# phylo42/IPK

Measured on AMD Instinct MI355X. Metric: scored phylo-k-mers/sec, higher is better.
Workload: dtype f32

## Files before the change

ipk_amd/csrc/dcla_device.hpp:

```cpp
#pragma once
#include <hip/hip_runtime.h>
#include <stdint.h>

namespace ipkgpu {

constexpr __host__ __device__ uint32_t ipow(uint32_t b, int e) { return e <= 0 ? 1u : b * ipow(b, e - 1); }
constexpr __host__ __device__ uint64_t ipow64(uint64_t b, int e) { return e <= 0 ? 1ull : b * ipow64(b, e - 1); }
constexpr __host__ __device__ uint32_t umin_c(uint32_t a, uint32_t b) { return a < b ? a : b; }
constexpr __host__ __device__ uint32_t umax_c(uint32_t a, uint32_t b) { return a > b ? a : b; }

constexpr uint32_t LIST_OVERFLOW = 0xFFFFFFFFu;

__host__ __device__ __forceinline__ uint32_t enc_score_bits(uint32_t u)
{
    return (u & 0x80000000u) ? ~u : (u | 0x80000000u);
}
__host__ __device__ __forceinline__ uint32_t dec_score_bits(uint32_t e)
{
    return (e & 0x80000000u) ? (e & 0x7fffffffu) : ~e;
}

__device__ __forceinline__ uint32_t lane_id() { return threadIdx.x & 63u; }
__device__ __forceinline__ uint64_t ballot64(bool p) { return __builtin_amdgcn_ballot_w64(p); }
__device__ __forceinline__ uint32_t to_sgpr(uint32_t x)
{
    uint32_t r;
    asm volatile("s_nop 0\n\tv_readfirstlane_b32 %0, %1" : "=s"(r) : "v"(x));
    return r;
}

typedef uint32_t u32x2_t __attribute__((ext_vector_type(2)));

#ifdef IPK_EXEC_ASSERT
__device__ unsigned int g_exec_violations;
#define IPK_ASSERT_FULL_EXEC() do { if (__builtin_amdgcn_ballot_w64(true) != ~0ull) atomicAdd(&g_exec_violations, 1u); } while (0)
#else
#define IPK_ASSERT_FULL_EXEC() ((void)0)
#endif

template <int IMM = 0>
__device__ __forceinline__ void store8_lanes(const void* uniform_base, uint32_t byte_off, uint32_t x, uint32_t y, uint64_t mask)
{
    u32x2_t data; data.x = x; data.y = y;
    IPK_ASSERT_FULL_EXEC();
    asm volatile("s_mov_b64 exec, %3\n\tglobal_store_dwordx2 %0, %1, %2 offset:%4\n\ts_mov_b64 exec, -1"
                 : : "v"(byte_off), "v"(data), "s"(uniform_base), "s"(mask), "n"(IMM) : "memory");
}
template <int IMM = 0>
__device__ __forceinline__ void store4_lanes(const void* uniform_base, uint32_t byte_off, uint32_t x, uint64_t mask)
{
    IPK_ASSERT_FULL_EXEC();
    asm volatile("s_mov_b64 exec, %3\n\tglobal_store_dword %0, %1, %2 offset:%4\n\ts_mov_b64 exec, -1"
                 : : "v"(byte_off), "v"(x), "s"(uniform_base), "s"(mask), "n"(IMM) : "memory");
}

__device__ __forceinline__ uint32_t mbcnt(uint64_t mask)
{
    return __builtin_amdgcn_mbcnt_hi((uint32_t)(mask >> 32), __builtin_amdgcn_mbcnt_lo((uint32_t)mask, 0u));
}
__device__ __forceinline__ void wave_lds_sync()
{
    __builtin_amdgcn_fence(__ATOMIC_RELEASE, "wavefront");
    __builtin_amdgcn_wave_barrier();
    __builtin_amdgcn_fence(__ATOMIC_ACQUIRE, "wavefront");
}

struct WinCtx {
    const float* cols;
    const float* best;
    uint32_t w;
    uint32_t lead_c = 0;
};

template <int SIGMA, int J, int H>
struct Direct {
    static __device__ __forceinline__ bool eval(const WinCtx& c, float eps, uint32_t cand, float& score)
    {
        if constexpr (H == 1) {
            score = c.cols[(c.w + J) * SIGMA + cand];
            return score > eps;
        } else {
            constexpr int HL = H / 2, HR = H - HL;
            const float eps_l = eps - (c.best[c.w + J + H] - c.best[c.w + J + HL]);
            const float eps_r = eps - (c.best[c.w + J + HL] - c.best[c.w + J]);
            constexpr uint32_t PR = ipow(SIGMA, HR);
            const uint32_t cl = cand / PR, cr = cand - cl * PR;
            float sl, sr;
            const bool okl = Direct<SIGMA, J, HL>::eval(c, eps_l, cl, sl);
            const bool okr = Direct<SIGMA, J + HL, HR>::eval(c, eps_r, cr, sr);
            score = sl + sr;
            return okl & okr & (score > eps);
        }
    }
};

template <int SIGMA, int H, int CAP>
struct Geo {
    static constexpr uint64_t FULL = ipow64(SIGMA, H);
    static constexpr uint32_t CAPH = (uint32_t)(FULL < (uint64_t)CAP ? FULL : (uint64_t)CAP);
    static constexpr bool DIRECT = FULL <= 64;
    static constexpr int HL = H / 2, HR = H - H / 2;
    static constexpr uint32_t scratch()
    {
        if constexpr (DIRECT) return 0;
        else {
            using GL = Geo<SIGMA, HL, CAP>;
            using GR = Geo<SIGMA, HR, CAP>;
            return umax_c(GL::CAPH + GL::scratch(), GL::CAPH + GR::CAPH + GR::scratch());
        }
    }
    static constexpr uint32_t SCRATCH = scratch();
};

template <int SIGMA, int K, int CAP>
constexpr uint32_t wave_scratch_entries() { return Geo<SIGMA, K, CAP>::SCRATCH; }

__device__ __forceinline__ void divmod_u(uint32_t idx, uint32_t d, float rcp_d, uint32_t& q, uint32_t& r)
{
    q = (uint32_t)(((float)idx + 0.5f) * rcp_d);
    int32_t rem = (int32_t)idx - (int32_t)(q * d);
    if (rem < 0) { q -= 1; rem += (int32_t)d; }
    else if (rem >= (int32_t)d) { q += 1; rem -= (int32_t)d; }
    r = (uint32_t)rem;
}

template <class F>
__device__ __forceinline__ void for_each_pair(const uint2* L, uint32_t nL, const uint2* R, uint32_t nR, F&& f)
{
    const uint32_t lane = lane_id();
// ... 111 lines not shown
```

ipk_amd/csrc/ipkgpu.hip:

```cpp
#include <cstring>
#include <hip/hip_runtime.h>
#include <rocprim/rocprim.hpp>

#include <algorithm>
#include <cmath>
#include <cstdarg>
#include <cstdio>
#include <cstring>
#include <new>
#include <string>
#include <type_traits>
#include <unordered_map>
#include <memory>
#include <vector>

#include "../../include/ipkgpu.h"
#include "dcla_device.hpp"
#include "kernels_score.hpp"
#include "kernels_quad.hpp"
#include "kernels_compact.hpp"
#include "kernels_keymajor.hpp"
#include "kernels_reduce_pipe.hpp"
#include "kernels_filter.hpp"
#include "kernels_dbfile.hpp"
// ... 1910 lines not shown
        HIP_TRY(ctx, ctx_alloc(ctx, (void**)&e->d_entries, 8));
        if (positions) {
            Geometry geo;
            RC_TRY(fill_geometry(ctx, sigma, k, 0, geo));
            if (lead != 0 || geo.xp_nb == 0)
                return fail(ctx, IPKGPU_ERR_INVALID, "no positioned database for sigma=%u k=%u: the call takes the exact partition, which needs more than 64 keys "
                                                     "and no key-range pass", sigma, k);
            HIP_TRY(ctx, ctx_alloc(ctx, (void**)&e->d_positions, 4));
        }
        HIP_TRY(ctx, hipMemsetAsync(e->d_counts, 0, (size_t)n_owners * e->slots * 4, ctx->stream));
        HIP_TRY(ctx, hipStreamSynchronize(ctx->stream));
        eg.r = nullptr;
        *out = e;
        return IPKGPU_OK;
    }
    Plan pl;
    RC_TRY(make_plan(ctx, logp_dev, n_mats, sites, sigma, mat_group, k, log_eps, pl, lead, lead_c, false, positions));
    HIP_TRY(ctx, hipSetDevice(ctx->device));
    if (positions) {
        std::vector<uint32_t> rank(n_mats), seen(pl.n_groups, 0);
        for (uint32_t i = 0; i < n_mats; ++i) rank[i] = seen[pl.slot_of[i]]++;
        const uint32_t most = *std::max_element(seen.begin(), seen.end());
        if ((uint64_t)most * pl.nwin >= 0xFFFFFFFFull) return fail(ctx, IPKGPU_ERR_INVALID, "too many windows per group for the position code (%u matrices x %u windows)", most, pl.nwin);
        RC_TRY(ensure(ctx, ctx->mrank, (size_t)n_mats * 4));
        HIP_TRY(ctx, hipMemcpy(ctx->mrank.p, rank.data(), (size_t)n_mats * 4, hipMemcpyHostToDevice));
        pl.mat_rank = ctx->mrank.as<uint32_t>();
    }
    const uint64_t T = pl.table_size;
    const uint32_t P = n_owners;
    const uint64_t slots = (T + P - 1) / P;
    const uint32_t n_groups = pl.n_groups;

    ipkgpu_parts* parts = new (std::nothrow) ipkgpu_parts();
    if (!parts) return fail(ctx, IPKGPU_ERR_NOMEM, "out of host memory");
    parts->ctx = ctx; parts->n_owners = P; parts->slots = slots;
    parts->lead = lead; parts->key_base = key_base; parts->sigma = sigma; parts->k = k;
    parts->owner_off.assign((size_t)P + 1, 0);
    struct Guard { ipkgpu_parts* r; ~Guard() { if (r) ipkgpu_parts_free(r); } } guard{parts};

    RC_TRY(ensure(ctx, ctx->branch, (size_t)n_groups * 4));
    ctx->h_branch = pl.group_ids;
    HIP_TRY(ctx, hipMemcpyAsync(ctx->branch.p, ctx->h_branch.data(), (size_t)n_groups * 4, hipMemcpyHostToDevice, ctx->stream));

    ctx->acc_main_ms = ctx->acc_reduce_ms = ctx->acc_count_ms = ctx->acc_write_ms = ctx->acc_km_ms = 0;
    Stopwatch sw(ctx->stream, &ctx->events);
    const int t_begin = sw.mark();
    RC_TRY(run_prefix(ctx, pl, logp_dev));
    const int t_pre = sw.mark();
    std::vector<std::pair<int, int>> ev_score, ev_compact, ev_km;
    std::pair<int, int> ev_keys{-1, -1};

    struct Batch { uint32_t* counts = nullptr; uint2* entries = nullptr; uint2* pentries = nullptr; std::vector<uint64_t> owner_off; };
    std::vector<Batch> batches;
    auto free_batches = [&]() { for (auto& b : batches) { ctx_release(ctx, b.counts); ctx_release(ctx, b.entries); ctx_release(ctx, b.pentries); } batches.clear(); };
    struct BGuard { decltype(free_batches)& f; ~BGuard() { f(); } } bguard{free_batches};

    const uint64_t n_slots_all = (uint64_t)P * slots;
    uint32_t gpb_now = (uint32_t)pl.gpb, gb = 0;
    for (uint32_t g0 = 0; g0 < n_groups; g0 += gb) {
        gb = std::min<uint32_t>(gpb_now, n_groups - g0);
        const int s0 = sw.mark();
        const int rcb = score_batch(ctx, pl, logp_dev, g0, gb, &parts->emitted, true);
        if (rcb == IPKGPU_RETRY_SMALLER) { gpb_now = std::max<uint32_t>(1, gb / 2); gb = 0; continue; }
        if (rcb) return rcb;
        const int s1 = sw.mark();
        ev_score.push_back({s0, s1});
        parts->score_launches += 1;

        batches.emplace_back();
        Batch& b = batches.back();
        HIP_TRY(ctx, ctx_alloc(ctx, (void**)&b.counts, n_slots_all * 4));
        HIP_TRY(ctx, hipMemsetAsync(b.counts, 0, n_slots_all * 4, ctx->stream));
        const uint32_t kmc_pass = (uint32_t)std::min<int64_t>(256, std::max<int64_t>(4, ctx->opt_kmc_pass > 0 ? ctx->opt_kmc_pass : IPK_KMC_PASS));
        const bool fast_c = ctx->table_compressed && 64ull * (ctx->mask_words / 2) * 8 < (1ull << 32);
        uint32_t* qpack = nullptr;
        if (fast_c) {
            RC_TRY(ensure(ctx, ctx->qpack, n_slots_all * 4));
            if (gb <= kmc_pass) qpack = ctx->qpack.as<uint32_t>();
        }
        if (ctx->mask_valid && (T + 31) / 32 >= (uint64_t)ctx->num_cu * 1024)
            hipLaunchKernelGGL(km_count_mask_kernel, dim3((uint32_t)(((T + 31) / 32 + 255) / 256)), dim3(256), 0, ctx->stream,
                               ctx->mask.as<uint32_t>(), ctx->mask_words, T, gb, P, slots, b.counts, qpack);
        else if (ctx->mask_valid)
            hipLaunchKernelGGL(km_count_mask_key_kernel, dim3((uint32_t)((T + 255) / 256)), dim3(256), 0, ctx->stream,
                               ctx->mask.as<uint32_t>(), ctx->mask_words, T, gb, P, slots, b.counts, qpack);
        else
            hipLaunchKernelGGL(km_count_kernel, dim3((uint32_t)((T + 255) / 256)), dim3(256), 0, ctx->stream,
                               ctx->table.as<uint32_t>(), T, gb, P, slots, b.counts);
        HIP_TRY(ctx, hipGetLastError());
        RC_TRY(ensure(ctx, ctx->offsets, (n_slots_all + 1) * 8));
        RC_TRY(scan_u32(ctx, b.counts, n_slots_all, ctx->offsets.as<uint64_t>()));
        RC_TRY(ensure(ctx, ctx->goff, ((size_t)P + 1) * 8));
        hipLaunchKernelGGL(gather_offsets_kernel, dim3((P + 1 + 255) / 256), dim3(256), 0, ctx->stream,
                           ctx->offsets.as<uint64_t>(), (uint32_t)slots, P + 1, ctx->goff.as<uint64_t>());
        HIP_TRY(ctx, hipGetLastError());
        b.owner_off.resize((size_t)P + 1);
        const bool rb_ok = P <= RB_OWNERS_MAX;
        uint64_t* h_off = rb_ok ? reinterpret_cast<uint64_t*>(ctx->h_rb) + RB_OWNER_OFF : b.owner_off.data();
        HIP_TRY(ctx, hipMemcpyAsync(h_off, ctx->goff.p, ((size_t)P + 1) * 8, hipMemcpyDeviceToHost, ctx->stream));

        const bool pre_keys = P == 1 && g0 == 0 && gb == n_groups && rb_ok && !(ctx->opt_flags & 64) &&
                              (slots <= (1ull << 24) || ctx->last_entries * 8 >= slots * 12 * 4);
        uint32_t* k_keys = nullptr; uint64_t* k_off = nullptr;
        struct KGuard { ipkgpu_ctx* c; uint32_t*& a; uint64_t*& b; ~KGuard() { ctx_release(c, a); ctx_release(c, b); } } kguard{ctx, k_keys, k_off};
        int kt0 = -1, kt1 = -1;
        if (pre_keys) {
            kt0 = sw.mark();
            RC_TRY(ensure(ctx, ctx->tmp_b, (slots + 1) * 8));
            RC_TRY(scan_nonzero_u32(ctx, b.counts, slots, ctx->tmp_b.as<uint64_t>()));
            HIP_TRY(ctx, hipMemcpyAsync(h_off + P + 1, ctx->tmp_b.as<uint64_t>() + slots, 8, hipMemcpyDeviceToHost, ctx->stream));
            HIP_TRY(ctx, ctx_alloc(ctx, (void**)&k_keys, slots * 4));
            HIP_TRY(ctx, ctx_alloc(ctx, (void**)&k_off, (slots + 1) * 8));
            const uint32_t nbk = (uint32_t)((slots + 1 + 255) / 256);
            if (sigma == 4)
                hipLaunchKernelGGL(merge_write_keys_kernel<4>, dim3(nbk), dim3(256), 0, ctx->stream, b.counts, ctx->tmp_b.as<uint64_t>(),
                                   ctx->offsets.as<uint64_t>(), slots, (uint32_t)key_base, 1u, (int)k, k_keys, k_off);
            else
                hipLaunchKernelGGL(merge_write_keys_kernel<20>, dim3(nbk), dim3(256), 0, ctx->stream, b.counts, ctx->tmp_b.as<uint64_t>(),
                                   ctx->offsets.as<uint64_t>(), slots, 0u, 1u, (int)k, k_keys, k_off);
            HIP_TRY(ctx, hipGetLastError());
            kt1 = sw.mark();
        }

        uint2* w_dst = nullptr; bool w_posv = false;
        auto comp_table_w = [&]() { CompTable c = comp_table(ctx); if (w_posv) c.vaddr = ctx->pvaddr.as<uint64_t>(); return c; };
        auto launch_writer = [&](uint64_t cap_e) -> int {
            uint2* const dst_entries = w_dst ? w_dst : b.entries;
            if (ctx->table_compressed) {
                uint64_t per_xcd = (((T + 63) / 64) + 7) / 8;
                const uint32_t rows_now = qpack ? gb : std::min<uint32_t>(gb, kmc_pass);
                const bool runs = !(ctx->opt_flags & 4096) && IPK_KMC_RUNS_DEFAULT && (rows_now <= 128 || (ctx->opt_flags & 8192));
                if (runs && (qpack || fast_c)) per_xcd = (kmc_runs(T, ctx->comp_tbl) + 7) / 8;
                if (qpack && runs)
                    KM_LAUNCH(km_write_c_run_kernel, KMC_CAP, comp_table_w(), T, gb, ctx->branch.as<uint32_t>() + g0, P, slots, b.counts,
                              qpack, ctx->offsets.as<uint64_t>(), dst_entries, cap_e);
                else if (qpack)
                    KM_LAUNCH(km_write_c_kernel, KMC_CAP, comp_table_w(), T, gb, ctx->branch.as<uint32_t>() + g0, P, slots, b.counts,
                              qpack, ctx->offsets.as<uint64_t>(), dst_entries, cap_e);
                else if (fast_c) {
                    RC_TRY(ensure(ctx, ctx->pcounts, n_slots_all * 4));
                    for (uint32_t p0 = 0; p0 < gb; p0 += kmc_pass) {
                        const uint32_t pg = std::min<uint32_t>(kmc_pass, gb - p0);
                        const uint32_t* pmask = ctx->mask.as<uint32_t>() + (size_t)p0 * ctx->mask_words;
                        if ((T + 31) / 32 >= (uint64_t)ctx->num_cu * 1024)
                            hipLaunchKernelGGL(km_count_mask_kernel, dim3((uint32_t)(((T + 31) / 32 + 255) / 256)), dim3(256), 0, ctx->stream,
                                               pmask, ctx->mask_words, T, pg, P, slots, ctx->pcounts.as<uint32_t>(), ctx->qpack.as<uint32_t>());
                        else
                            hipLaunchKernelGGL(km_count_mask_key_kernel, dim3((uint32_t)((T + 255) / 256)), dim3(256), 0, ctx->stream,
                                               pmask, ctx->mask_words, T, pg, P, slots, ctx->pcounts.as<uint32_t>(), ctx->qpack.as<uint32_t>());
                        HIP_TRY(ctx, hipGetLastError());
                        CompTable ctp = comp_table_w();
                        ctp.mask = pmask;
                        ctp.vaddr += (size_t)p0 * (ctx->mask_words / 2);
                        ctp.rank += (size_t)p0 * (ctx->mask_words / 2);
                        if (runs)
                            KM_LAUNCH(km_write_c_run_kernel, KMC_CAP, ctp, T, pg, ctx->branch.as<uint32_t>() + g0 + p0, P, slots, ctx->pcounts.as<uint32_t>(),
                                      ctx->qpack.as<uint32_t>(), ctx->offsets.as<uint64_t>(), dst_entries, cap_e);
                        else
                            KM_LAUNCH(km_write_c_kernel, KMC_CAP, ctp, T, pg, ctx->branch.as<uint32_t>() + g0 + p0, P, slots, ctx->pcounts.as<uint32_t>(),
                                      ctx->qpack.as<uint32_t>(), ctx->offsets.as<uint64_t>(), dst_entries, cap_e);
                        HIP_TRY(ctx, hipGetLastError());
                    }
                } else if (positions)
                    return fail(ctx, IPKGPU_ERR_INVALID, "a positioned database of this many key slots per group would take the generic key-major writer, which carries no positions");
                else
                    hipLaunchKernelGGL(km_write_c_generic_kernel, dim3((uint32_t)((((T + 63) / 64 + 7) / 8) * 8)), dim3(256), 0, ctx->stream,
                                       comp_table(ctx), T, gb, ctx->branch.as<uint32_t>() + g0, P, slots,
                                       ctx->offsets.as<uint64_t>(), b.entries, cap_e);
            } else if ((ctx->opt_flags & 512) || (gb < 96 && !(ctx->opt_flags & 1024)))
                hipLaunchKernelGGL(km_write_kernel, dim3((uint32_t)((T + 63) / 64)), dim3(256), 0, ctx->stream,
                                   ctx->table.as<uint32_t>(), T, gb, ctx->branch.as<uint32_t>() + g0, P, slots,
                                   ctx->offsets.as<uint64_t>(), b.entries, cap_e);
            else
                hipLaunchKernelGGL(km_write_lines_kernel, dim3((uint32_t)((T + 63) / 64)), dim3(256), 0, ctx->stream,
                                   ctx->table.as<uint32_t>(), T, gb, ctx->branch.as<uint32_t>() + g0, P, slots,
                                   ctx->offsets.as<uint64_t>(), b.entries, cap_e);
            HIP_TRY(ctx, hipGetLastError());
            return IPKGPU_OK;
        };
        uint64_t cap_e = 0;
        const bool spec_e = rb_ok && ctx->last_gb > 0 && ctx->last_entries > 0 && !(ctx->opt_flags & 64) && !positions;
        int km0 = -1, km1 = -1;
        if (spec_e) {
            const uint64_t est = (uint64_t)((unsigned __int128)ctx->last_entries * gb / ctx->last_gb);
            size_t got = 0;
            if (ctx_alloc_atleast(ctx, (void**)&b.entries, est * 8, (est + est / 20 + 4096) * 8, &got) == hipSuccess) cap_e = got / 8;
            else { (void)hipGetLastError(); b.entries = nullptr; }
        }
        if (cap_e) { km0 = sw.mark(); RC_TRY(launch_writer(cap_e)); km1 = sw.mark(); }
        HIP_TRY(ctx, hipStreamSynchronize(ctx->stream));
        const int rcf = ctx->pend.active ? score_batch_finish(ctx, pl, g0, gb, &parts->emitted) : IPKGPU_OK;
        if (rcf == IPKGPU_RETRY_SMALLER || rcf == IPKGPU_RETRY_AGAIN) {
            ctx_release(ctx, b.counts); ctx_release(ctx, b.entries);
            batches.pop_back();
            ev_score.pop_back(); parts->score_launches -= 1;
            if (rcf == IPKGPU_RETRY_SMALLER) gpb_now = std::max<uint32_t>(1, gb / 2);
            gb = 0;
            continue;
        }
        if (rcf) return rcf;
        if (rb_ok) memcpy(b.owner_off.data(), h_off, ((size_t)P + 1) * 8);
        if (b.owner_off[P] > cap_e || cap_e == 0) {
            ctx_release(ctx, b.entries); b.entries = nullptr;
            HIP_TRY(ctx, ctx_alloc(ctx, (void**)&b.entries, std::max<uint64_t>(b.owner_off[P], 1) * 8));
            const uint64_t n_e = std::max<uint64_t>(b.owner_off[P], 1);
            km0 = sw.mark();
            if (positions) {
                if (!ctx->table_compressed) return fail(ctx, IPKGPU_ERR_INVALID, "internal: a positioned call ended in dense tables");
                const size_t cur_bytes = (n_slots_all + 1) * 8;
                RC_TRY(ensure(ctx, ctx->cursnap, cur_bytes));
                HIP_TRY(ctx, hipMemcpyAsync(ctx->cursnap.p, ctx->offsets.p, cur_bytes, hipMemcpyDeviceToDevice, ctx->stream));
                RC_TRY(launch_writer(n_e));
                HIP_TRY(ctx, hipMemcpyAsync(ctx->offsets.p, ctx->cursnap.p, cur_bytes, hipMemcpyDeviceToDevice, ctx->stream));
                HIP_TRY(ctx, ctx_alloc(ctx, (void**)&b.pentries, n_e * 8));
                w_dst = b.pentries; w_posv = true;
                RC_TRY(launch_writer(n_e));
                w_dst = nullptr; w_posv = false;
            } else
                RC_TRY(launch_writer(n_e));
            km1 = sw.mark();
        }
        ctx->last_entries = b.owner_off[P]; ctx->last_gb = gb;
        if (pre_keys) {
            parts->pre_keys = k_keys; parts->pre_key_off = k_off; parts->pre_n_keys = h_off[P + 1];
            k_keys = nullptr; k_off = nullptr;
            ev_keys = {kt0, kt1};
        }
        ev_km.push_back({km0, km1});
        ev_compact.push_back({s1, km1});
    }

    auto extract_positions = [&](const uint2* src, uint64_t n, uint32_t* dst) -> int {
        if (!n) return IPKGPU_OK;
        hipLaunchKernelGGL(extract_positions_kernel, dim3((uint32_t)((n + 255) / 256)), dim3(256), 0, ctx->stream, src, n, dst);
        HIP_TRY(ctx, hipGetLastError());
        return IPKGPU_OK;
    };
    if (batches.size() == 1) {
        parts->d_counts = batches[0].counts; parts->d_entries = batches[0].entries;
        parts->owner_off = batches[0].owner_off;
        batches[0].counts = nullptr; batches[0].entries = nullptr;
        if (positions) {
            const int m0 = sw.mark();
            HIP_TRY(ctx, ctx_alloc(ctx, (void**)&parts->d_positions, std::max<uint64_t>(parts->owner_off[P], 1) * 4));
            RC_TRY(extract_positions(batches[0].pentries, parts->owner_off[P], parts->d_positions));
            ev_compact.push_back({m0, sw.mark()});
        }
    } else {
        const int m0 = sw.mark();
        const uint32_t S = (uint32_t)batches.size();
        HIP_TRY(ctx, ctx_alloc(ctx, (void**)&parts->d_counts, n_slots_all * 4));
        uint64_t grand = 0;
        for (auto& b : batches) grand += b.owner_off[P];
        HIP_TRY(ctx, ctx_alloc(ctx, (void**)&parts->d_entries, std::max<uint64_t>(grand, 1) * 8));
        if (positions) HIP_TRY(ctx, ctx_alloc(ctx, (void**)&parts->d_positions, std::max<uint64_t>(grand, 1) * 4));
        uint64_t done = 0;
        int rc = IPKGPU_OK;
        for (uint32_t o = 0; o < P && rc == IPKGPU_OK; ++o) {
            std::vector<const uint32_t*> crow(S);
// ... 921 lines not shown
```

ipk_amd/csrc/kernels_keymajor.hpp:

```cpp
#pragma once
#include <type_traits>
#include "dcla_device.hpp"
#include "comp_table.hpp"

namespace ipkgpu {

typedef const uint32_t __attribute__((address_space(1)))* global_u32_ptr;


__global__ __launch_bounds__(256) void km_count_kernel(const uint32_t* __restrict__ table, uint64_t T, uint32_t G,
                                                       uint32_t P, uint64_t slots, uint32_t* __restrict__ counts)
{
    const uint64_t x = (uint64_t)blockIdx.x * 256 + threadIdx.x;
    if (x >= T) return;
    uint32_t c = 0;
    const uint32_t* t = table + x;
    uint32_t g = 0;
    for (; g + 4 <= G; g += 4) {
        const uint32_t v0 = t[(size_t)(g + 0) * T], v1 = t[(size_t)(g + 1) * T];
        const uint32_t v2 = t[(size_t)(g + 2) * T], v3 = t[(size_t)(g + 3) * T];
        c += (v0 != 0u) + (v1 != 0u) + (v2 != 0u) + (v3 != 0u);
    }
    for (; g < G; ++g) c += (t[(size_t)g * T] != 0u);
    const uint64_t o = x % P, q = x / P;
    counts[o * slots + q] = c;
}

__global__ __launch_bounds__(256) void km_count_mask_kernel(const uint32_t* __restrict__ mask, uint64_t W, uint64_t T,
                                                            uint32_t G, uint32_t P, uint64_t slots, uint32_t* __restrict__ counts,
                                                            uint32_t* __restrict__ qpack)
{
    const uint64_t w = (uint64_t)blockIdx.x * 256 + threadIdx.x;
    if (w * 32 >= T) return;
    uint32_t plane[8] = {0, 0, 0, 0, 0, 0, 0, 0};
    uint32_t total[32], pack[32];
#pragma unroll
    for (int b = 0; b < 32; ++b) { total[b] = 0; pack[b] = 0; }
    const uint32_t* m = mask + w;
    const uint32_t step = qpack ? (G + 3) / 4 : 255u;
    uint32_t q = 0;
    for (uint32_t g0 = 0; g0 < G; g0 += step, ++q) {
        const uint32_t g1 = min(G, g0 + step);
        uint32_t g = g0;
        for (; g + 8 <= g1; g += 8) {
            uint32_t v[8];
#pragma unroll
            for (int u = 0; u < 8; ++u) v[u] = m[(size_t)(g + u) * W];
#pragma unroll
            for (int u = 0; u < 8; ++u) {
                uint32_t carry = v[u];
#pragma unroll
                for (int p = 0; p < 8; ++p) { const uint32_t t = plane[p] & carry; plane[p] ^= carry; carry = t; }
            }
        }
        for (; g < g1; ++g) {
            uint32_t carry = m[(size_t)g * W];
#pragma unroll
            for (int p = 0; p < 8; ++p) { const uint32_t t = plane[p] & carry; plane[p] ^= carry; carry = t; }
        }
#pragma unroll
        for (int b = 0; b < 32; ++b) {
            uint32_t c = 0;
#pragma unroll
            for (int p = 0; p < 8; ++p) c |= ((plane[p] >> b) & 1u) << p;
            total[b] += c;
            pack[b] |= c << ((8u * q) & 31u);
        }
#pragma unroll
        for (int p = 0; p < 8; ++p) plane[p] = 0;
    }
    if (P == 1 && w * 32 + 32 <= T) {
        uint4* c4 = reinterpret_cast<uint4*>(counts + w * 32);
        uint4* q4 = reinterpret_cast<uint4*>(qpack + w * 32);
#pragma unroll
        for (int b = 0; b < 32; b += 4) {
            c4[b >> 2] = make_uint4(total[b], total[b + 1], total[b + 2], total[b + 3]);
            if (qpack) q4[b >> 2] = make_uint4(pack[b], pack[b + 1], pack[b + 2], pack[b + 3]);
        }
        return;
    }
#pragma unroll
    for (int b = 0; b < 32; ++b) {
        const uint64_t x = w * 32 + b;
        if (x < T) {
            const uint64_t idx = (x % P) * slots + x / P;
            counts[idx] = total[b];
            if (qpack) qpack[idx] = pack[b];
        }
    }
}

__global__ __launch_bounds__(256) void km_count_mask_key_kernel(const uint32_t* __restrict__ mask, uint64_t W, uint64_t T,
                                                                uint32_t G, uint32_t P, uint64_t slots, uint32_t* __restrict__ counts,
                                                                uint32_t* __restrict__ qpack)
{
    const uint64_t x = (uint64_t)blockIdx.x * 256 + threadIdx.x;
    if (x >= T) return;
    const uint32_t* m = mask + (x >> 5);
    const uint32_t sh = (uint32_t)x & 31u;
    const uint32_t step = qpack ? (G + 3) / 4 : G;
    uint32_t total = 0, pack = 0, q = 0;
    for (uint32_t g0 = 0; g0 < G; g0 += step, ++q) {
        const uint32_t g1 = min(G, g0 + step);
        uint32_t c = 0, g = g0;
        for (; g + 16 <= g1; g += 16) {
            uint32_t v[16];
#pragma unroll
            for (int u = 0; u < 16; ++u) v[u] = m[(size_t)(g + u) * W];
#pragma unroll
            for (int u = 0; u < 16; ++u) c += (v[u] >> sh) & 1u;
        }
        for (; g < g1; ++g) c += (m[(size_t)g * W] >> sh) & 1u;
        total += c;
        pack |= c << ((8u * q) & 31u);
    }
    const uint64_t idx = (x % P) * slots + x / P;
    counts[idx] = total;
    if (qpack) qpack[idx] = pack;
}

constexpr uint32_t SCAN_BLOCK = 4096;

__global__ __launch_bounds__(256) void scan_block_sums_kernel(const uint32_t* __restrict__ in, uint64_t n,
                                                              uint32_t* __restrict__ sums)
{
    __shared__ uint32_t wsum[4];
    const uint64_t s0 = (uint64_t)blockIdx.x * SCAN_BLOCK;
    const uint32_t m = (uint32_t)min((uint64_t)SCAN_BLOCK, n - s0);
    uint32_t acc = 0;
    for (uint32_t i = threadIdx.x; i < m; i += 256) acc += in[s0 + i];
    for (int o = 32; o > 0; o >>= 1) acc += __shfl_down(acc, o);
    if (lane_id() == 0) wsum[threadIdx.x >> 6] = acc;
    __syncthreads();
    if (threadIdx.x == 0) sums[blockIdx.x] = wsum[0] + wsum[1] + wsum[2] + wsum[3];
}

__global__ __launch_bounds__(256) void scan_apply_kernel(const uint32_t* __restrict__ in, uint64_t n,
                                                         const uint64_t* __restrict__ block_off,
                                                         uint64_t* __restrict__ out)
{
    __shared__ uint32_t tsum[256];
    const uint64_t s0 = (uint64_t)blockIdx.x * SCAN_BLOCK;
    const uint32_t m = (uint32_t)min((uint64_t)SCAN_BLOCK, n - s0);
    constexpr uint32_t PER = SCAN_BLOCK / 256;
    const uint32_t lo = threadIdx.x * PER;
    uint32_t v[PER];
    uint32_t acc = 0;
#pragma unroll
    for (uint32_t i = 0; i < PER; ++i) { v[i] = (lo + i < m) ? in[s0 + lo + i] : 0u; acc += v[i]; }
    tsum[threadIdx.x] = acc;
    __syncthreads();
    uint32_t x = acc;
    for (uint32_t d = 1; d < 256; d <<= 1) {
        const uint32_t y = (threadIdx.x >= d) ? tsum[threadIdx.x - d] : 0u;
        __syncthreads();
        x += y; tsum[threadIdx.x] = x;
        __syncthreads();
    }
    uint64_t run = block_off[blockIdx.x] + (uint64_t)(x - acc);
#pragma unroll
    for (uint32_t i = 0; i < PER; ++i) { if (lo + i < m) out[s0 + lo + i] = run; run += v[i]; }
    if (blockIdx.x == gridDim.x - 1 && threadIdx.x == 255) out[n] = block_off[blockIdx.x] + (uint64_t)x;
}

__global__ __launch_bounds__(256) void km_write_kernel(const uint32_t* __restrict__ table, uint64_t T, uint32_t G,
                                                       const uint32_t* __restrict__ branch_of_group, uint32_t P,
                                                       uint64_t slots, uint64_t* __restrict__ cursor,
                                                       uint2* __restrict__ entries, uint64_t cap_entries)
{
    __shared__ uint32_t tile[64][65];
    if (cursor[(uint64_t)P * slots] > cap_entries) return;
    const uint64_t x0 = (uint64_t)blockIdx.x * 64;
    const uint32_t wave = (uint32_t)__builtin_amdgcn_readfirstlane((int)(threadIdx.x >> 6)), lane = lane_id();
    size_t cidx = 0;
    uint64_t cur = 0;
    const bool mine = lane < 16 && x0 + wave + 4u * lane < T;
    if (mine) {
        const uint64_t x = x0 + wave + 4u * lane;
        cidx = (size_t)((x % P) * slots + x / P);
        cur = cursor[cidx];
    }
    uint2* dst[16];
#pragma unroll
    for (int t = 0; t < 16; ++t) {
        const uint32_t lo = (uint32_t)__builtin_amdgcn_readlane((int)(uint32_t)cur, t);
        const uint32_t hi = (uint32_t)__builtin_amdgcn_readlane((int)(uint32_t)(cur >> 32), t);
        dst[t] = entries + (((uint64_t)hi << 32) | lo);
    }
    const uint32_t xl = threadIdx.x & 63u;
    const bool xok = x0 + xl < T;
    for (uint32_t g0 = 0; g0 < G; g0 += 64) {
        uint32_t v[16];
#pragma unroll
        for (uint32_t u = 0; u < 16; ++u) {
            const uint32_t gl = wave + 4u * u;
            v[u] = 0;
#ifdef IPK_KMW_NOLOAD
            if (g0 + gl < G && xok) v[u] = (uint32_t)(g0 + gl + x0 + xl) | 0x80000000u;
#else
            if (g0 + gl < G && xok) v[u] = table[(size_t)(g0 + gl) * T + x0 + xl];
#endif
        }
        const uint32_t br = (g0 + lane < G) ? branch_of_group[g0 + lane] : 0u;
        __syncthreads();
#pragma unroll
        for (uint32_t u = 0; u < 16; ++u) tile[wave + 4u * u][xl] = v[u];
        __syncthreads();
        uint32_t wq[16];
#pragma unroll
        for (int t = 0; t < 16; ++t) wq[t] = tile[lane][wave + 4u * (uint32_t)t];
#pragma unroll
        for (int t = 0; t < 16; ++t) {
            const uint32_t w = wq[t];
            const uint64_t cm = ballot64(w != 0u);
#if defined(IPK_KMW_ALIGNED)
            store8_lanes(reinterpret_cast<const void*>(reinterpret_cast<uintptr_t>(dst[t]) & ~(uintptr_t)511), lane_id() << 3, br, dec_score_bits(w), ~0ull);
#elif defined(IPK_KMW_NOSTORE)
            store8_lanes(dst[t], mbcnt(cm) << 3, br, dec_score_bits(w), cm & (ballot64(w == 0x12345u) != 0 ? ~0ull : 0ull));
#else
            store8_lanes(dst[t], mbcnt(cm) << 3, br, dec_score_bits(w), cm);
#endif
            dst[t] += __popcll(cm);
        }
    }
    uint64_t fin = 0;
#pragma unroll
    for (int t = 0; t < 16; ++t)
        if (lane == (uint32_t)t) fin = (uint64_t)(dst[t] - entries);
    if (mine) cursor[cidx] = fin;
}

__global__ __launch_bounds__(256) void km_write_lines_kernel(const uint32_t* __restrict__ table, uint64_t T, uint32_t G,
                                                             const uint32_t* __restrict__ branch_of_group, uint32_t P,
                                                             uint64_t slots, uint64_t* __restrict__ cursor,
                                                             uint2* __restrict__ entries, uint64_t cap_entries)
{
    __shared__ uint32_t tile[64][65];
    __shared__ uint2 work[4][80];
    if (cursor[(uint64_t)P * slots] > cap_entries) return;
    const uint64_t x0 = (uint64_t)blockIdx.x * 64;
    const uint32_t wave = (uint32_t)__builtin_amdgcn_readfirstlane((int)(threadIdx.x >> 6)), lane = lane_id();
    size_t cidx = 0;
    uint64_t cur = 0;
    const bool mine = lane < 16 && x0 + wave + 4u * lane < T;
    if (mine) {
        const uint64_t x = x0 + wave + 4u * lane;
        cidx = (size_t)((x % P) * slots + x / P);
        cur = cursor[cidx];
    }
    uint64_t pos[16];
    uint32_t tl[16];
    uint32_t tbr[16], tsc[16];
#pragma unroll
    for (int t = 0; t < 16; ++t) {
        const uint32_t lo = (uint32_t)__builtin_amdgcn_readlane((int)(uint32_t)cur, t);
        const uint32_t hi = (uint32_t)__builtin_amdgcn_readlane((int)(uint32_t)(cur >> 32), t);
        pos[t] = ((uint64_t)hi << 32) | lo;
        tl[t] = 0; tbr[t] = 0; tsc[t] = 0;
    }
    uint2* const wk = work[wave];
    const uint32_t lane8 = lane << 3;
    const uint32_t xl = threadIdx.x & 63u;
    const bool xok = x0 + xl < T;
    for (uint32_t g0 = 0; g0 < G; g0 += 64) {
        uint32_t v[16];
#pragma unroll
        for (uint32_t u = 0; u < 16; ++u) {
            const uint32_t gl = wave + 4u * u;
            v[u] = 0;
            if (g0 + gl < G && xok) v[u] = table[(size_t)(g0 + gl) * T + x0 + xl];
        }
        const uint32_t br = (g0 + lane < G) ? branch_of_group[g0 + lane] : 0u;
        __syncthreads();
#pragma unroll
        for (uint32_t u = 0; u < 16; ++u) tile[wave + 4u * u][xl] = v[u];
        __syncthreads();
        uint32_t wq[16];
#pragma unroll
        for (int t = 0; t < 16; ++t) wq[t] = tile[lane][wave + 4u * (uint32_t)t];
#pragma unroll
        for (int t = 0; t < 16; ++t) {
            const uint32_t w = wq[t];
            const uint64_t cm = ballot64(w != 0u);
            const uint32_t n = (uint32_t)__popcll(cm);
            const uint32_t tlt = tl[t];
            const uint32_t total = tlt + n;
            wave_lds_sync();
            if (lane < tlt) wk[lane] = make_uint2(tbr[t], tsc[t]);
            if (w != 0u) wk[tlt + mbcnt(cm)] = make_uint2(br, dec_score_bits(w));
            wave_lds_sync();
            const uint32_t over = (uint32_t)((pos[t] + total) & 15u);
            const uint32_t cut = over <= total ? total - over : 0u;
            const uint32_t rem = total - cut;
            const uint2 e0 = wk[lane], e1 = wk[min(64u + lane, 79u)], er = wk[min(cut + lane, 79u)];
            if (cut) {
                uint2* const d = entries + pos[t];
                const uint64_t m0 = cut >= 64 ? ~0ull : ((1ull << cut) - 1ull);
                store8_lanes(d, lane8, e0.x, e0.y, m0);
                if (cut > 64) store8_lanes<512>(d, lane8, e1.x, e1.y, (1ull << (cut - 64)) - 1ull);
            }
            tbr[t] = er.x; tsc[t] = er.y;
            tl[t] = rem;
            pos[t] += cut;
        }
    }
    uint64_t fin = 0;
#pragma unroll
    for (int t = 0; t < 16; ++t) {
        if (tl[t]) store8_lanes(entries + pos[t], lane8, tbr[t], tsc[t], (1ull << tl[t]) - 1ull);
        if (lane == (uint32_t)t) fin = pos[t] + tl[t];
    }
    if (mine) cursor[cidx] = fin;
}

__global__ __launch_bounds__(256) void km_write_c_generic_kernel(CompTable ct, uint64_t T, uint32_t G,
                                                         const uint32_t* __restrict__ branch_of_group, uint32_t P,
                                                         uint64_t slots, uint64_t* __restrict__ cursor,
                                                         uint2* __restrict__ entries, uint64_t cap_entries)
{
    __shared__ uint32_t tile[64][65];
    __shared__ uint64_t run[64];
    if (cursor[(uint64_t)P * slots] > cap_entries) return;
    __shared__ uint64_t row_mask[64];
    __shared__ const uint32_t* row_vals[64];
    const uint64_t nblocks = (T + 63) / 64, per_xcd = (nblocks + 7) / 8;
    const uint64_t kb = (uint64_t)(blockIdx.x & 7u) * per_xcd + (blockIdx.x >> 3);
    if ((blockIdx.x >> 3) >= per_xcd || kb >= nblocks) return;
    const uint64_t x0 = kb * 64;
    const uint32_t b = (uint32_t)(x0 / ct.TBL);
    const uint32_t wave = threadIdx.x >> 6, lane = lane_id();
    if (threadIdx.x < 64) {
        const uint64_t x = x0 + threadIdx.x;
        run[threadIdx.x] = (x < T) ? cursor[(x % P) * slots + x / P] : 0;
    }
    for (uint32_t g0 = 0; g0 < G; g0 += 64) {
        __syncthreads();
        if (threadIdx.x < 64) {
            const uint32_t g = g0 + threadIdx.x;
            uint64_t m = 0;
            const uint32_t* vp = nullptr;
            if (g < G) {
                const uint32_t* mw = ct.mask + (size_t)g * ct.mask_words + 2 * kb;
                m = (uint64_t)mw[0] | ((uint64_t)mw[1] << 32);
                vp = reinterpret_cast<const uint32_t*>(ct.pool + ct.off[((size_t)g * ct.NB + b) * ct.stride]) +
                     ct.rank[(size_t)g * (ct.mask_words / 2) + kb];
            }
            row_mask[threadIdx.x] = m; row_vals[threadIdx.x] = vp;
        }
        __syncthreads();
        for (uint32_t i = threadIdx.x; i < 4096; i += 256) {
            const uint32_t gl = i >> 6, xl = i & 63u;
            const uint64_t m = row_mask[gl];
            uint32_t v = 0;
            if ((m >> xl) & 1ull) v = ((global_u32_ptr)row_vals[gl])[(uint32_t)__popcll(m & ((1ull << xl) - 1ull))];
            tile[gl][xl] = v;
        }
        __syncthreads();
        const uint32_t br = (g0 + lane < G) ? branch_of_group[g0 + lane] : 0u;
        for (uint32_t xl = wave; xl < 64; xl += 4) {
            const uint32_t v = tile[lane][xl];
            const uint64_t m = __ballot(v != 0u);
            if (m == 0) continue;
            const uint64_t base = run[xl];
            if (v != 0u) entries[base + mbcnt(m)] = make_uint2(br, dec_score_bits(v));
            if (lane == 0) run[xl] = base + (uint64_t)__popcll(m);
        }
    }
    __syncthreads();
    if (threadIdx.x < 64) {
        const uint64_t x = x0 + threadIdx.x;
        if (x < T) cursor[(x % P) * slots + x / P] = run[threadIdx.x];
    }
}

template <typename T>
__device__ __forceinline__ T uniform_load(const T* p)
{
    return *(const __attribute__((address_space(4))) T*)(uintptr_t)(p);
}
__device__ __forceinline__ uint32_t lds_address(const void* p)
{
    return (uint32_t)(uintptr_t)(const __attribute__((address_space(3))) void*)(p);
// ... 547 lines not shown
```

Measured before the change: 140.5 billion.

## Count mask bits with bit-sliced slice kernel and add nontemporal line stores

Replaces the per-key mask counting kernel with a block kernel where each thread reads whole 32-bit mask words over a slice of groups. It accumulates the bits with a bit-sliced vertical counter (eight planes of carry-save adds), then merges the per-key counts through LDS atomics before writing counts and quarter-packed counts. This cuts the repeated strided reads of the same mask word by 32 threads and the per-bit shift work. Separately, the line-writer kernel now issues nontemporal stores for aligned full lines by default (opt-out flag), to reduce cache pollution from streaming entry writes. The new counter adds LDS atomics and register pressure from the plane arrays.

```diff
diff --git a/ipk_amd/csrc/dcla_device.hpp b/ipk_amd/csrc/dcla_device.hpp
--- a/ipk_amd/csrc/dcla_device.hpp
+++ b/ipk_amd/csrc/dcla_device.hpp
@@ -38,13 +38,17 @@
 #define IPK_ASSERT_FULL_EXEC() ((void)0)
 #endif
 
-template <int IMM = 0>
+template <int IMM = 0, bool NTS = false>
 __device__ __forceinline__ void store8_lanes(const void* uniform_base, uint32_t byte_off, uint32_t x, uint32_t y, uint64_t mask)
 {
     u32x2_t data; data.x = x; data.y = y;
     IPK_ASSERT_FULL_EXEC();
-    asm volatile("s_mov_b64 exec, %3\n\tglobal_store_dwordx2 %0, %1, %2 offset:%4\n\ts_mov_b64 exec, -1"
-                 : : "v"(byte_off), "v"(data), "s"(uniform_base), "s"(mask), "n"(IMM) : "memory");
+    if constexpr (NTS)
+        asm volatile("s_mov_b64 exec, %3\n\tglobal_store_dwordx2 %0, %1, %2 offset:%4 nt\n\ts_mov_b64 exec, -1"
+                     : : "v"(byte_off), "v"(data), "s"(uniform_base), "s"(mask), "n"(IMM) : "memory");
+    else
+        asm volatile("s_mov_b64 exec, %3\n\tglobal_store_dwordx2 %0, %1, %2 offset:%4\n\ts_mov_b64 exec, -1"
+                     : : "v"(byte_off), "v"(data), "s"(uniform_base), "s"(mask), "n"(IMM) : "memory");
 }
 template <int IMM = 0>
 __device__ __forceinline__ void store4_lanes(const void* uniform_base, uint32_t byte_off, uint32_t x, uint64_t mask)
diff --git a/ipk_amd/csrc/ipkgpu.hip b/ipk_amd/csrc/ipkgpu.hip
--- a/ipk_amd/csrc/ipkgpu.hip
+++ b/ipk_amd/csrc/ipkgpu.hip
@@ -2016,7 +2016,7 @@
             hipLaunchKernelGGL(km_count_mask_kernel, dim3((uint32_t)(((T + 31) / 32 + 255) / 256)), dim3(256), 0, ctx->stream,
                                ctx->mask.as<uint32_t>(), ctx->mask_words, T, gb, P, slots, b.counts, qpack);
         else if (ctx->mask_valid)
-            hipLaunchKernelGGL(km_count_mask_key_kernel, dim3((uint32_t)((T + 255) / 256)), dim3(256), 0, ctx->stream,
+            hipLaunchKernelGGL(km_count_mask_slice_kernel, dim3((uint32_t)(((T + 31) / 32 + KMS_WORDS - 1) / KMS_WORDS)), dim3(KMS_WORDS * KMS_SLICES), 0, ctx->stream,
                                ctx->mask.as<uint32_t>(), ctx->mask_words, T, gb, P, slots, b.counts, qpack);
         else
             hipLaunchKernelGGL(km_count_kernel, dim3((uint32_t)((T + 255) / 256)), dim3(256), 0, ctx->stream,
@@ -2080,7 +2080,7 @@
                             hipLaunchKernelGGL(km_count_mask_kernel, dim3((uint32_t)(((T + 31) / 32 + 255) / 256)), dim3(256), 0, ctx->stream,
                                                pmask, ctx->mask_words, T, pg, P, slots, ctx->pcounts.as<uint32_t>(), ctx->qpack.as<uint32_t>());
                         else
-                            hipLaunchKernelGGL(km_count_mask_key_kernel, dim3((uint32_t)((T + 255) / 256)), dim3(256), 0, ctx->stream,
+                            hipLaunchKernelGGL(km_count_mask_slice_kernel, dim3((uint32_t)(((T + 31) / 32 + KMS_WORDS - 1) / KMS_WORDS)), dim3(KMS_WORDS * KMS_SLICES), 0, ctx->stream,
                                                pmask, ctx->mask_words, T, pg, P, slots, ctx->pcounts.as<uint32_t>(), ctx->qpack.as<uint32_t>());
                         HIP_TRY(ctx, hipGetLastError());
                         CompTable ctp = comp_table_w();
@@ -2105,10 +2105,12 @@
                 hipLaunchKernelGGL(km_write_kernel, dim3((uint32_t)((T + 63) / 64)), dim3(256), 0, ctx->stream,
                                    ctx->table.as<uint32_t>(), T, gb, ctx->branch.as<uint32_t>() + g0, P, slots,
                                    ctx->offsets.as<uint64_t>(), b.entries, cap_e);
-            else
-                hipLaunchKernelGGL(km_write_lines_kernel, dim3((uint32_t)((T + 63) / 64)), dim3(256), 0, ctx->stream,
+            else {
+                const auto lines = (ctx->opt_flags & 16384) ? km_write_lines_kernel<false> : km_write_lines_kernel<true>;
+                hipLaunchKernelGGL(lines, dim3((uint32_t)((T + 63) / 64)), dim3(256), 0, ctx->stream,
                                    ctx->table.as<uint32_t>(), T, gb, ctx->branch.as<uint32_t>() + g0, P, slots,
                                    ctx->offsets.as<uint64_t>(), b.entries, cap_e);
+            }
             HIP_TRY(ctx, hipGetLastError());
             return IPKGPU_OK;
         };
diff --git a/ipk_amd/csrc/kernels_keymajor.hpp b/ipk_amd/csrc/kernels_keymajor.hpp
--- a/ipk_amd/csrc/kernels_keymajor.hpp
+++ b/ipk_amd/csrc/kernels_keymajor.hpp
@@ -90,33 +90,65 @@
     }
 }
 
-__global__ __launch_bounds__(256) void km_count_mask_key_kernel(const uint32_t* __restrict__ mask, uint64_t W, uint64_t T,
-                                                                uint32_t G, uint32_t P, uint64_t slots, uint32_t* __restrict__ counts,
-                                                                uint32_t* __restrict__ qpack)
-{
-    const uint64_t x = (uint64_t)blockIdx.x * 256 + threadIdx.x;
-    if (x >= T) return;
-    const uint32_t* m = mask + (x >> 5);
-    const uint32_t sh = (uint32_t)x & 31u;
-    const uint32_t step = qpack ? (G + 3) / 4 : G;
-    uint32_t total = 0, pack = 0, q = 0;
-    for (uint32_t g0 = 0; g0 < G; g0 += step, ++q) {
-        const uint32_t g1 = min(G, g0 + step);
-        uint32_t c = 0, g = g0;
-        for (; g + 16 <= g1; g += 16) {
-            uint32_t v[16];
-#pragma unroll
-            for (int u = 0; u < 16; ++u) v[u] = m[(size_t)(g + u) * W];
-#pragma unroll
-            for (int u = 0; u < 16; ++u) c += (v[u] >> sh) & 1u;
-        }
-        for (; g < g1; ++g) c += (m[(size_t)g * W] >> sh) & 1u;
-        total += c;
-        pack |= c << ((8u * q) & 31u);
-    }
-    const uint64_t idx = (x % P) * slots + x / P;
-    counts[idx] = total;
-    if (qpack) qpack[idx] = pack;
+constexpr uint32_t KMS_WORDS = 32, KMS_SLICES = 16;
+__global__ __launch_bounds__(KMS_WORDS * KMS_SLICES) void km_count_mask_slice_kernel(const uint32_t* __restrict__ mask, uint64_t W, uint64_t T,
+                                                                  uint32_t G, uint32_t P, uint64_t slots, uint32_t* __restrict__ counts,
+                                                                  uint32_t* __restrict__ qpack)
+{
+    constexpr uint32_t NT = KMS_WORDS * KMS_SLICES, NK = KMS_WORDS * 32;
+    __shared__ uint32_t tot[32 * (KMS_WORDS + 1)], pk[32 * (KMS_WORDS + 1)];
+    for (uint32_t i = threadIdx.x; i < 32 * (KMS_WORDS + 1); i += NT) { tot[i] = 0; pk[i] = 0; }
+    __syncthreads();
+    const uint32_t wl = threadIdx.x % KMS_WORDS, s = threadIdx.x / KMS_WORDS;
+    const uint64_t w = (uint64_t)blockIdx.x * KMS_WORDS + wl;
+    const uint32_t step = (G + 3) / 4, q = s >> 2;
+    const uint32_t q0 = min(G, q * step), q1 = min(G, q0 + step);
+    const uint32_t sub = (q1 - q0 + 3) / 4;
+    const uint32_t s0 = min(q1, q0 + (s & 3u) * sub), s1 = min(q1, s0 + sub);
+    if (w * 32 < T) {
+        const uint32_t* m = mask + w;
+        for (uint32_t g0 = s0; g0 < s1; g0 += 255) {
+            const uint32_t g1 = min(s1, g0 + 255u);
+            uint32_t plane[8] = {0, 0, 0, 0, 0, 0, 0, 0};
+            uint32_t g = g0;
+            for (; g + 8 <= g1; g += 8) {
+                uint32_t v[8];
+#pragma unroll
+                for (int u = 0; u < 8; ++u) v[u] = m[(size_t)(g + u) * W];
+#pragma unroll
+                for (int u = 0; u < 8; ++u) {
+                    uint32_t carry = v[u];
+#pragma unroll
+                    for (int p = 0; p < 8; ++p) { const uint32_t t = plane[p] & carry; plane[p] ^= carry; carry = t; }
+                }
+            }
+            for (; g < g1; ++g) {
+                uint32_t carry = m[(size_t)g * W];
+#pragma unroll
+                for (int p = 0; p < 8; ++p) { const uint32_t t = plane[p] & carry; plane[p] ^= carry; carry = t; }
+            }
+#pragma unroll
+            for (int b = 0; b < 32; ++b) {
+                uint32_t c = 0;
+#pragma unroll
+                for (int p = 0; p < 8; ++p) c |= ((plane[p] >> b) & 1u) << p;
+                if (c) {
+                    atomicAdd(&tot[b * (KMS_WORDS + 1) + wl], c);
+                    if (qpack) atomicAdd(&pk[b * (KMS_WORDS + 1) + wl], c << (8u * q));
+                }
+            }
+        }
+    }
+    __syncthreads();
+    for (uint32_t i = threadIdx.x; i < NK; i += NT) {
+        const uint64_t x = (uint64_t)blockIdx.x * NK + i;
+        if (x < T) {
+            const uint64_t idx = (x % P) * slots + x / P;
+            const uint32_t at = (i & 31u) * (KMS_WORDS + 1) + (i >> 5);
+            counts[idx] = tot[at];
+            if (qpack) qpack[idx] = pk[at];
+        }
+    }
 }
 
 constexpr uint32_t SCAN_BLOCK = 4096;
@@ -230,6 +262,7 @@
     if (mine) cursor[cidx] = fin;
 }
 
+template <bool NTS>
 __global__ __launch_bounds__(256) void km_write_lines_kernel(const uint32_t* __restrict__ table, uint64_t T, uint32_t G,
                                                              const uint32_t* __restrict__ branch_of_group, uint32_t P,
                                                              uint64_t slots, uint64_t* __restrict__ cursor,
@@ -296,8 +329,11 @@
             if (cut) {
                 uint2* const d = entries + pos[t];
                 const uint64_t m0 = cut >= 64 ? ~0ull : ((1ull << cut) - 1ull);
-                store8_lanes(d, lane8, e0.x, e0.y, m0);
-                if (cut > 64) store8_lanes<512>(d, lane8, e1.x, e1.y, (1ull << (cut - 64)) - 1ull);
+                auto put = [&](auto nt) {
+                    store8_lanes<0, decltype(nt)::value>(d, lane8, e0.x, e0.y, m0);
+                    if (cut > 64) store8_lanes<512, decltype(nt)::value>(d, lane8, e1.x, e1.y, (1ull << (cut - 64)) - 1ull);
+                };
+                if (NTS && (pos[t] & 15u) == 0) put(std::true_type{}); else put(std::false_type{});
             }
             tbr[t] = er.x; tsc[t] = er.y;
             tl[t] = rem;
```

New measurement: 143.4 billion, median of 6. 2.0% higher.
